# lachinov/brats2019

Measured on AMD Instinct MI355X. Metric: volumes_per_sec_fwd_bwd_128cubed_x4ch, higher is better.
Workload: dtype bf16

## Files before the change

### brats2019_amd/_lib.py

```python
from __future__ import annotations

import ctypes as C
import os

import torch

_PKG = os.path.dirname(os.path.abspath(__file__))
LIB_PATH = os.environ.get("RU_LIB_PATH") or os.path.join(_PKG, "lib", "libresunet_hip.so")

_lib = None
PRECISIONS = {"f32": 0, "bf16x3": 1}
GRAD_PRECISIONS = {"bf16x3": 1, "bf16": 2}
FUSE_GN_BWD_STATS, FUSE_GN_BWD_APPLY, FUSE_SIDE_STREAM, FUSE_BATCH_WREDUCE, FUSE_TAIL_FINALIZE, FUSE_PW_DGRAD = 1, 2, 4, 8, 16, 32

_vp, _f, _d, _i, _sz = C.c_void_p, C.c_float, C.c_double, C.c_int, C.c_size_t

SIGNATURES = {
    "ru_last_error": (C.c_char_p, []),
    "ru_version": (_i, []),
    "ru_device_ok": (_i, []),
    "ru_conv3d_workspace_bytes": (_sz, [_i] * 7),
    "ru_conv3d_fwd": (_i, [_vp, _vp, _vp, _vp] + [_i] * 7 + [_vp, _sz, _vp]),
    "ru_conv3d_bwd_data": (_i, [_vp, _vp, _vp] + [_i] * 7 + [_vp, _sz, _vp]),
    "ru_conv3d_fwd_p": (_i, [_vp, _vp, _vp, _vp] + [_i] * 8 + [_vp, _sz, _vp]),
# ... 48 lines not shown
    "ru_comm_destroy": (_i, [_vp]),
    "ru_comm_rank": (_i, [_vp]),
    "ru_comm_world": (_i, [_vp]),
    "ru_allreduce": (_i, [_vp, _vp, _sz, _i, _vp]),
    "ru_comm_group_begin": (_i, []),
    "ru_comm_group_end": (_i, []),
    "ru_tta_merge": (_i, [_vp, _i, C.c_uint, _vp, _vp, _vp, _i, _i, _i, _i, _vp]),
    "ru_compose_labels": (_i, [_vp, _vp, C.c_ulonglong, _vp, _sz, _vp]),
    "ru_dice_counts": (_i, [_vp, _vp, _vp, _i, _i, _sz, _vp]),
    "ru_dice_accumulate": (_i, [_vp, _vp, _i, _i, _i, _vp]),
    "ru_hausdorff_workspace_bytes": (_sz, [_i] * 6),
    "ru_hausdorff_sq": (_i, [_vp, _vp] + [_i] * 6 + [_vp, _vp, _sz, _vp]),
    "ru_hausdorff_accumulate": (_i, [_vp, _vp] + [_i] * 4 + [_vp]),
    "ru_label_confusion": (_i, [_vp, _vp, _i, _i, _i, _sz, _vp, _vp, _vp]),
    "ru_overlap_accumulate": (_i, [_vp, _i, _i, _i, _i, _vp, _vp, _vp]),
    "ru_dice1d_accumulate": (_i, [_vp, _vp, _i, _i, _i, _vp]),
    "ru_rmse_accumulate": (_i, [_vp, _vp, _vp]),
    "ru_tile_gather": (_i, [_vp, _vp] + [_i] * 6 + [C.POINTER(_i), _i, _i, _i, _vp]),
    "ru_tile_scatter": (_i, [_vp, _vp] + [_i] * 6 + [C.POINTER(_i), _i, _i, _i, C.POINTER(_i), C.POINTER(_i), _vp]),
    "ru_case_bbox": (_i, [_vp, _vp, _i, _i, _i, _i, _vp]),
    "ru_case_workspace_bytes": (_sz, [_i, _i, _i, _i]),
    "ru_case_stats": (_i, [_vp, _vp, _i, _i, _i, _i, C.POINTER(_i), C.POINTER(_i), _vp, _sz, _vp]),
    "ru_case_prepare": (_i, [_vp, _vp, _vp, _i, _i, _i, _i, C.POINTER(_i), C.POINTER(_i), C.POINTER(_i), C.POINTER(_i), _i, C.c_uint, _vp]),
    "ru_tta_merge_box": (_i, [_vp, _i, C.c_uint, _vp, _vp, _vp, _i, _i, _i, _i, C.POINTER(_i), C.POINTER(_i), _vp]),
    "ru_cc_workspace_bytes": (_sz, [_i, _i, _i]),
    "ru_cc_reject": (_i, [_vp, _i, _i, _i, _d, _vp, _sz, _vp]),
    "ru_paste_labels": (_i, [_vp, _vp, _i, _i, _i, C.POINTER(_i), C.POINTER(_i), _vp]),
    "ru_zscore_workspace_bytes": (_sz, [_i, _sz]),
    "ru_zscore_stats": (_i, [_vp, _vp, _i, _sz, _vp, _sz, _vp]),
    "ru_augment_patch": (_i, [_vp, _vp, _vp, _vp, _i, _i, _i, _i, _vp, _vp, _vp, _i, _vp, _vp, _vp, _vp, _vp]),
    "ru_layout_convert": (_i, [_vp, _vp, _i, _i, _sz, _i, _vp]),
    "ru_upsample2x_trilinear_fwd_l": (_i, [_vp, _vp] + [_i] * 5 + [_f, _vp]),
    "ru_upsample2x_trilinear_bwd_l": (_i, [_vp, _vp] + [_i] * 5 + [_vp]),
    "ru_conv3d_fwd_l": (_i, [_vp, _vp, _vp, _vp] + [_i] * 7 + [_vp, _sz, _vp]),
    "ru_conv3d_bwd_weight_l": (_i, [_vp, _vp, _vp] + [_i] * 7 + [_vp, _sz, _vp]),
}


CRIT_KINDS = {"Dice_loss_joint": 0, "BCE_Loss": 1, "MSE_Loss": 2, "CE_Loss": 3, "Dice1D": 4, "GDL_joint": 5, "sens_loss_joint": 6,
              "Dice_loss_separate": 7}
CRIT_MOMENTS, CRIT_MAX_TERMS = 7, 8
CRIT_MASK_LOGS, CRIT_MASK_ALL = (1 << 4) | (1 << 5), 0x7F
CRIT_M_D2 = 6

CONF_PROB, CONF_LABEL, OVERLAP_MAX_LABELS = 0, 1, 8
OVERLAP_MODES = {"itk": 0, "wt": 1, "validate": 2}


class CritTerm(C.Structure):
    _fields_ = [("kind", _i), ("weight", _d), ("priority", _d), ("bg_weight", _d)]


def load():
    global _lib
    if _lib is not None:
        return _lib
    if not os.path.exists(LIB_PATH):
        raise RuntimeError(
            "libresunet_hip.so not found at %s -- build it with `python -m brats2019_amd.build` "
            "(hipcc, gfx950).  There is no CPU fallback for this path." % LIB_PATH)
    lib = C.CDLL(LIB_PATH)
    for name, (res, args) in SIGNATURES.items():
        if os.environ.get("RU_LIB_PATH") and not hasattr(lib, name):
            continue
        fn = getattr(lib, name)
        fn.restype = res
# ... 45 lines not shown
```

### brats2019_amd/csrc/engine.hip

```cpp
#include "ru_common.h"

#include <vector>
#include <math.h>
#include <stdlib.h>
#include <string.h>

#include <string>
#include <vector>

namespace ru {

static thread_local char g_err[512] = "";
void set_error(const char* fmt, ...) {
    va_list ap;
    va_start(ap, fmt);
    vsnprintf(g_err, sizeof(g_err), fmt, ap);
    va_end(ap);
}
int hip_fail(hipError_t e, const char* what) {
    set_error("%s: %s", what, hipGetErrorString(e));
    return RU_EHIP;
}

constexpr float kSlope = 1e-2f;
// ... 614 lines not shown
    }
    const float* cur = stem_fused ? h->y0 : h->t0;
    h->first_s.assign(h->first_blocks.size(), BlockSave());
    for (size_t j = 0; j < h->first_blocks.size(); ++j) {
        rc = block_fwd(h, params, A, s, h->first_blocks[j], cur, N, Dl[0], Hl[0], Wl[0], h->first_s[j], &cur, (stem_fused && j == 0) ? &h->g0 : nullptr);
        if (rc) return rc;
    }
    h->skips.assign(depth - 1, nullptr);
    h->enc_s.assign(depth - 1, {});
    for (int i = 0; i < depth - 1; ++i) {
        h->skips[i] = cur;
        h->enc_s[i].assign(h->enc_blocks[i].size(), BlockSave());
        for (size_t j = 0; j < h->enc_blocks[i].size(); ++j) {
            const int lv = j == 0 ? i : i + 1;
            rc = block_fwd(h, params, A, s, h->enc_blocks[i][j], cur, N, Dl[lv], Hl[lv], Wl[lv], h->enc_s[i][j], &cur);
            if (rc) return rc;
        }
    }
    h->dstage.assign(depth - 1, DecSave());
    h->dec_s.assign(depth - 1, {});
    for (int i = depth - 2; i >= 0; --i) {
        DecSave& ds = h->dstage[i];
        ds.level = i;
        ds.z = cur;
        ds.skip = h->skips[i];
        const int Ci = h->ch[i], Cc = h->ch[i + 1];
        const bool recycle = !h->training;
        float* c_early = recycle ? A.alloc((size_t)N * Ci * Vl(i)) : nullptr;
        const size_t dmark = A.off;
        if (!h->c16) {
            ds.u = A.alloc((size_t)N * Cc * Vl(i));
            RU_RUN(up2_fwd_launch(cur, ds.u, N, Cc, Dl[i + 1], Hl[i + 1], Wl[i + 1], s));
        }
        ds.v = A.alloc((size_t)N * Ci * Vl(i));
        Conv1Args c1{};
        c1.x0 = ds.u; c1.C0 = Cc; c1.y = ds.v; c1.out_slope = kSlope;
        c1.N = N; c1.Cout = Ci; c1.V = Vl(i);
        ds.c = recycle ? c_early : A.alloc((size_t)N * Ci * Vl(i));
        Conv1Args c2{};
        c2.x0 = ds.skip; c2.C0 = Ci; c2.x1 = ds.v; c2.C1 = Ci;
        c2.y = ds.c; c2.out_slope = 1.f; c2.N = N; c2.Cout = Ci; c2.V = Vl(i);
        if (h->c16) {
            float* zc = A.alloc((size_t)N * Ci * Vl(i + 1));
            c1.x0 = cur; c1.y = zc; c1.out_slope = 1.f; c1.V = Vl(i + 1);
            c1.wT = P(h, params, h->up_w[i]); c1.ldw = Cc;
            RU_RUN(conv1_16_launch(c1, s));
            RU_RUN(up2_fwd16_launch(zc, ds.v, N, Ci, Dl[i + 1], Hl[i + 1], Wl[i + 1], kSlope, s));
            c2.wT = P(h, params, h->dec1_w[i]); c2.ldw = 2 * Ci;
            RU_RUN(conv1_16_launch(c2, s));
        } else {
            c1.wT = h->pack + h->pk_upT[i]; c1.ldw = Ci;
            RU_RUN(conv1_launch(c1, s));
            c2.wT = h->pack + h->pk_decT[i]; c2.ldw = Ci;
            RU_RUN(conv1_launch(c2, s));
        }
        if (recycle) A.rewind(dmark);
        cur = ds.c;
        h->dec_s[i].assign(h->dec_blocks[i].size(), BlockSave());
        for (size_t j = 0; j < h->dec_blocks[i].size(); ++j) {
            const bool defer = i == 0 && j + 1 == h->dec_blocks[i].size() && h->c16 &&
                               (h->precision == RU_PREC_BF16X3 ? conv3_sb_head_takes_residual(N, C0, h->nout, Dl[0], Hl[0], Wl[0])
                                                               : (!h->training && conv3_f32c_head_takes_residual(C0, h->nout, Wl[0])));
            rc = block_fwd(h, params, A, s, h->dec_blocks[i][j], cur, N, Dl[i], Hl[i], Wl[i], h->dec_s[i][j], &cur, nullptr, defer);
            if (rc) return rc;
            if (defer) head_block = &h->dec_s[i][j];
        }
    }
    h->head_in = cur;
    t_hint_c = C0;
    float* pdst = probs_out;
    h->probs = probs_out;
    Conv3Args a{};
    a.x = cur; a.wp = h->pack + h->pk_out; a.bias = P(h, params, h->conv_out_b); a.y = pdst; a.sigmoid = 1;
    a.mode = h->precision; a.wfrag = h->fpack + h->fk_out; a.in_c16 = h->c16;
    a.N = N; a.Cin = C0; a.Cout = h->nout; a.D = Dl[0]; a.H = Hl[0]; a.W = Wl[0];
    if (head_block) {
        a.x = head_block->y2; a.in_scale = head_block->g2.scale; a.in_shift = head_block->g2.shift; a.in_slope = kSlope; a.in_res = head_block->x;
        a.in_sum_out = head_block->out;
    }
    RU_RUN(conv3_launch(a, s));
    if (!A.dry) { h->packed_params = h->training ? nullptr : params; h->packed_base = h->pack; h->packed_prec = h->precision; h->packed_c16 = h->c16; h->pack_sig = conv3_sb_switch_signature(); }
    return RU_OK;
// ... 828 lines not shown

extern "C" int ru_tta_merge(const float* probs, int K, unsigned flips, float* mean_out, unsigned char* mask, unsigned long long* counts,
                            int C, int D, int H, int W, ru_stream_t stream) {
    RU_REQUIRE(probs && mask && counts, "ru_tta_merge: null argument");
    return tta_merge_launch(probs, K, flips, mean_out, mask, counts, C, D, H, W, (hipStream_t)stream);
}
extern "C" int ru_compose_labels(const unsigned char* mask, const unsigned long long* counts, unsigned long long et_min, unsigned char* labels,
                                 size_t V, ru_stream_t stream) {
    RU_REQUIRE(mask && counts && labels, "ru_compose_labels: null argument");
    return compose_labels_launch(mask, counts, et_min, labels, V, (hipStream_t)stream);
}

extern "C" int ru_dice_accumulate(const unsigned long long* counts, double* acc, int N, int C, int nacc, ru_stream_t stream) {
    return dice_accumulate_launch(counts, acc, N, C, nacc, (hipStream_t)stream);
}
extern "C" int ru_dice_counts(const float* p, const float* g, unsigned long long* counts, int N, int C, size_t V, ru_stream_t stream) {
    RU_REQUIRE(p && g && counts && N > 0 && C > 0, "ru_dice_counts: bad argument");
    return dice_counts_launch(p, g, counts, N * C, V, (hipStream_t)stream);
}

extern "C" int ru_layout_convert(const float* src, float* dst, int N, int C, size_t V, int to_c16, ru_stream_t stream) {
    RU_REQUIRE(src && dst && N > 0, "ru_layout_convert: bad argument");
    return layout_convert_launch(src, dst, N, C, V, to_c16, (hipStream_t)stream);
}

extern "C" int ru_upsample2x_trilinear_fwd_l(const float* x, float* y, int N, int C, int D, int H, int W, float out_slope, ru_stream_t stream) {
    RU_REQUIRE(x && y && N > 0 && C > 0 && D > 0 && H > 0 && W > 0, "ru_upsample2x_trilinear_fwd_l: bad argument");
    return up2_fwd16_launch(x, y, N, C, D, H, W, out_slope, (hipStream_t)stream);
}
extern "C" int ru_upsample2x_trilinear_bwd_l(const float* dy, float* dx, int N, int C, int D, int H, int W, ru_stream_t stream) {
    RU_REQUIRE(dy && dx && N > 0 && C > 0 && D > 0 && H > 0 && W > 0, "ru_upsample2x_trilinear_bwd_l: bad argument");
    return up2_bwd16_launch(dy, dx, N, C, D, H, W, (hipStream_t)stream);
}
extern "C" int ru_conv3d_fwd_l(const float* x, const float* w, const float* bias, float* y, int N, int Cin, int Cout, int D, int H, int W,
                               int flags, void* ws, size_t ws_bytes, ru_stream_t stream) {
    RU_REQUIRE(x && w && y, "ru_conv3d_fwd_l: null argument");
    hipStream_t s = (hipStream_t)stream;
    WsCarver C(ws, ws_bytes);
    Conv3Args a{};
    void* wf = C.take(conv3_sb_frag_bytes(Cin, Cout) / 4 + 64);
    RU_WS_OK(C);
    const bool f32 = (flags & 16) != 0;
    a.products = (flags & 32) ? 2 : 0;
    RU_REQUIRE(!f32 || ((flags & 3) != 0 && !(flags & (4 | 8))), "ru_conv3d_fwd_l: the exact-f32 form needs a voxel-major side and takes neither the 4-channel copy nor a split-form input");
    const bool gop = (flags & 64) && !f32 && (flags & 3) == 3 && !(flags & (4 | 8)) && !bias && conv3_mxg_usable(N, Cin, Cout, D, H, W);
    int rc = f32 ? conv3_f32c_pack_weights(w, wf, Cin, Cout, 0, s) : conv3_sb_pack_weights(w, wf, Cin, Cout, 0, s, gop);
    if (rc) return rc;
    a.mode = f32 ? RU_PREC_F32 : RU_PREC_BF16X3; a.wfrag = wf;
    a.in_c16 = flags & 1; a.out_c16 = (flags >> 1) & 1;
    a.in_s16 = (flags >> 3) & 1;
    RU_REQUIRE(!a.in_s16 || a.in_c16, "ru_conv3d_fwd_l: the split form is a voxel-major layout");
    a.x = x; a.bias = bias; a.y = y; a.N = N; a.Cin = Cin; a.Cout = Cout; a.D = D; a.H = H; a.W = W;
    if (gop) {
        const size_t nvox = (size_t)N * D * H * W;
        float* g16 = C.take(nvox * 16);
        RU_WS_OK(C);
        rc = conv3_mxg_split_launch(x, g16, nvox, s);
        if (rc) return rc;
        a.x = g16; a.in_s16 = 1; a.in_g16 = 1; a.products = 0;
    }
    if (flags & 4) {
        RU_REQUIRE(!(flags & 1) && conv3_sb4_usable(N, Cin, Cout, D, H, W), "ru_conv3d_fwd_l: shape does not fit the 4-channel kernel");
        const size_t V = (size_t)D * H * W;
        float* x4 = C.take((size_t)N * 4 * V);
        void* wf4 = C.take(conv3_sb4_frag_bytes(Cout) / 4 + 64);
        RU_WS_OK(C);
// ... 44 lines not shown
```

### brats2019_amd/csrc/pointwise_c16.hip

```cpp
#include "pw_helpers.hpp"
#include "fin_tail.hpp"
#include <type_traits>
#include <stdlib.h>

namespace ru {

typedef float f32x4_c16 __attribute__((ext_vector_type(4)));
template <int I, int N, class F> __device__ __forceinline__ void static_for_c1_impl(F&& f) {
    if constexpr (I < N) { f(std::integral_constant<int, I>{}); static_for_c1_impl<I + 1, N>(f); }
}
template <int N, class F> __device__ __forceinline__ void static_for_c1(F&& f) { static_for_c1_impl<0, N>(f); }

static inline dim3 c16_grid(size_t V, int blocks_nc, unsigned cap = 2048) {
    size_t bx = (V * 4 + 255) / 256;
    if (bx > cap) bx = cap;
    if (bx < 1) bx = 1;
    return dim3((unsigned)bx, (unsigned)blocks_nc);
}

template <int RES, bool NT = false>
__global__ __launch_bounds__(256) void gn_apply16_kernel(const float* __restrict__ x, const float* __restrict__ scale, const float* __restrict__ shift,
                                                         const float* __restrict__ res, float* __restrict__ y, int C, size_t V, float slope,
                                                         const float* __restrict__ rscale, const float* __restrict__ rshift, float rslope) {
    const int nb = blockIdx.y, CB = C >> 4;
// ... 164 lines not shown
        pw_split8(o, hi, lo);
        op[v * 4 + hf] = hi;
        op[v * 4 + 2 + hf] = lo;
    }
}
int gn_bwd_apply16_launch(const float* x, const float* dy, const float* scale, const float* shift, const float* coef, float slope, float* dx,
                          int N, int C, size_t V, int split, hipStream_t s) {
    RU_REQUIRE(C % 16 == 0, "gn_bwd_apply16: C must be a multiple of 16");
    if (split) {
        size_t bx = (V * 2 + 255) / 256;
        if (bx > 2048) bx = 2048;
        hipLaunchKernelGGL(gn_bwd_apply16_split_kernel, dim3((unsigned)bx, (unsigned)(N * (C / 16))), dim3(256), 0, s, x, dy, scale, shift, coef, slope, dx, C, V);
    } else {
        hipLaunchKernelGGL(gn_bwd_apply16_kernel, c16_grid(V, N * (C / 16)), dim3(256), 0, s, x, dy, scale, shift, coef, slope, dx, C, V);
    }
    RU_CHECK_LAUNCH("gn_bwd_apply16_kernel");
    return RU_OK;
}

__global__ __launch_bounds__(256) void up2_fwd16_kernel(const float* __restrict__ x, float* __restrict__ y, int D, int H, int W, float slope) {
    const int Do = 2 * D, Ho = 2 * H, Wo = 2 * W;
    const size_t nb = blockIdx.y;
    const size_t Vi = (size_t)D * H * W, Vo = Vi * 8;
    const float4* xp = reinterpret_cast<const float4*>(x) + nb * Vi * 4;
    float4* yp = reinterpret_cast<float4*>(y) + nb * Vo * 4;
    const bool nt_out = (size_t)gridDim.y * Vo * 16 * sizeof(float) >= ((size_t)128 << 20);
    const size_t total = (size_t)(D + 1) * (H + 1) * Wo * 4;
    for (size_t f = (size_t)blockIdx.x * 256 + threadIdx.x; f < total; f += (size_t)gridDim.x * 256) {
        const int q = (int)(f & 3);
        size_t r = f >> 2;
        const int xo = (int)(r % Wo); r /= Wo;
        const int ky = (int)(r % (H + 1)) - 1;
        const int kz = (int)(r / (H + 1)) - 1;
        int x0, x1; float lx0, lx1;
        up2_src(xo, W, x0, x1, lx0, lx1);
        const int zA = kz < 0 ? 0 : kz, zB = kz + 1 > D - 1 ? D - 1 : kz + 1;
        const int yA = ky < 0 ? 0 : ky, yB = ky + 1 > H - 1 ? H - 1 : ky + 1;
        const size_t rAA = ((size_t)zA * H + yA) * W, rAB = ((size_t)zA * H + yB) * W, rBA = ((size_t)zB * H + yA) * W, rBB = ((size_t)zB * H + yB) * W;
        const float4 a00 = xp[(rAA + x0) * 4 + q], b00 = xp[(rAA + x1) * 4 + q];
        const float4 a01 = xp[(rAB + x0) * 4 + q], b01 = xp[(rAB + x1) * 4 + q];
        const float4 a10 = xp[(rBA + x0) * 4 + q], b10 = xp[(rBA + x1) * 4 + q];
        const float4 a11 = xp[(rBB + x0) * 4 + q], b11 = xp[(rBB + x1) * 4 + q];
        float4 e00, e01, e10, e11;
#define RU_UPX(c) e00.c = lx0 * a00.c + lx1 * b00.c; e01.c = lx0 * a01.c + lx1 * b01.c; e10.c = lx0 * a10.c + lx1 * b10.c; e11.c = lx0 * a11.c + lx1 * b11.c
        RU_UPX(x); RU_UPX(y); RU_UPX(z); RU_UPX(w);
#undef RU_UPX
#pragma unroll
        for (int dz = 0; dz < 2; ++dz) {
            const int zo = 2 * kz + 1 + dz;
            if (zo < 0 || zo >= Do) continue;
            int z0, z1; float lz0, lz1;
            up2_src(zo, D, z0, z1, lz0, lz1);
#pragma unroll
            for (int dy = 0; dy < 2; ++dy) {
                const int yo = 2 * ky + 1 + dy;
                if (yo < 0 || yo >= Ho) continue;
                int y0, y1; float ly0, ly1;
                up2_src(yo, H, y0, y1, ly0, ly1);
                float4 o;
#define RU_UP2(c) o.c = lrelu(lz0 * (ly0 * e00.c + ly1 * e01.c) + lz1 * (ly0 * e10.c + ly1 * e11.c), slope)
                RU_UP2(x); RU_UP2(y); RU_UP2(z); RU_UP2(w);
#undef RU_UP2
                if (nt_out) __builtin_nontemporal_store(f32x4_c16{o.x, o.y, o.z, o.w}, reinterpret_cast<f32x4_c16*>(yp + (((size_t)zo * Ho + yo) * Wo + xo) * 4 + q));
                else yp[(((size_t)zo * Ho + yo) * Wo + xo) * 4 + q] = o;
            }
        }
    }
}
int up2_fwd16_launch(const float* x, float* y, int N, int C, int D, int H, int W, float slope, hipStream_t s) {
    RU_REQUIRE(C % 16 == 0, "up2_fwd16: C must be a multiple of 16");
    const size_t total = (size_t)(D + 1) * (H + 1) * (2 * W) * 4;
    size_t bx = (total + 255) / 256;
    if (bx > 16384) bx = 16384;
    hipLaunchKernelGGL(up2_fwd16_kernel, dim3((unsigned)bx, (unsigned)(N * (C / 16))), dim3(256), 0, s, x, y, D, H, W, slope);
    RU_CHECK_LAUNCH("up2_fwd16_kernel");
    return RU_OK;
}

#ifndef RU_UP2B_ZC
#define RU_UP2B_ZC 8
#endif
constexpr int UP2B_ZC = RU_UP2B_ZC;
__global__ __launch_bounds__(256) void up2_bwd16_kernel(const float* __restrict__ dy, float* __restrict__ dx, int D, int H, int W) {
    const int Do = 2 * D, Ho = 2 * H, Wo = 2 * W;
    const size_t nb = blockIdx.y;
    const size_t Vi = (size_t)D * H * W, Vo = Vi * 8;
    const float4* dp = reinterpret_cast<const float4*>(dy) + nb * Vo * 4;
    float4* op = reinterpret_cast<float4*>(dx) + nb * Vi * 4;
    const int nch = (D + UP2B_ZC - 1) / UP2B_ZC;
    const size_t total = (size_t)nch * H * W * 4;
    for (size_t f = (size_t)blockIdx.x * 256 + threadIdx.x; f < total; f += (size_t)gridDim.x * 256) {
        const int q = (int)(f & 3);
        size_t r = f >> 2;
        const int kx = (int)(r % W); r /= W;
        const int ky = (int)(r % H);
        const int k0 = (int)(r / H) * UP2B_ZC;
        const int k1 = k0 + UP2B_ZC < D ? k0 + UP2B_ZC : D;
        float wy[4], wx[4];
        size_t oy[4], ox[4];
#pragma unroll
        for (int t = 0; t < 4; ++t) {
            const int y = 2 * ky - 1 + t, xx = 2 * kx - 1 + t;
            wy[t] = (y >= 0 && y < Ho) ? up2_coef(y, H, ky) : 0.f;
            wx[t] = (xx >= 0 && xx < Wo) ? up2_coef(xx, W, kx) : 0.f;
            oy[t] = (size_t)(y < 0 ? 0 : (y >= Ho ? Ho - 1 : y)) * Wo;
            ox[t] = (size_t)(xx < 0 ? 0 : (xx >= Wo ? Wo - 1 : xx)) * 4 + q;
        }
        float4 accP = make_float4(0.f, 0.f, 0.f, 0.f), accC = accP;
// ... 426 lines not shown
```

### brats2019_amd/csrc/pw_helpers.hpp

```cpp
#pragma once
#include "ru_common.h"

namespace ru {

__device__ __forceinline__ float wave_sum(float v) {
#pragma unroll
    for (int o = 32; o > 0; o >>= 1) v += __shfl_xor(v, o);
    return v;
}
__device__ __forceinline__ double wave_sum_d(double v) {
#pragma unroll
    for (int o = 32; o > 0; o >>= 1) v += __shfl_xor(v, o);
    return v;
}
__device__ __forceinline__ float block_sum(float v, float* buf) {
    v = wave_sum(v);
    __syncthreads();
    if ((threadIdx.x & 63) == 0) buf[threadIdx.x >> 6] = v;
    __syncthreads();
    return buf[0] + buf[1] + buf[2] + buf[3];
}
__device__ __forceinline__ double block_sum_d(double v, double* buf) {
    v = wave_sum_d(v);
    __syncthreads();
    if ((threadIdx.x & 63) == 0) buf[threadIdx.x >> 6] = v;
    __syncthreads();
    return buf[0] + buf[1] + buf[2] + buf[3];
}
__device__ __forceinline__ float lrelu(float v, float slope) { return v > 0.f ? v : v * slope; }

static inline unsigned grid1d(size_t n, int per_block, unsigned cap = 1u << 20) {
    size_t b = (n + per_block - 1) / per_block;
    if (b < 1) b = 1;
    return (unsigned)(b > cap ? cap : b);
}

typedef __bf16 pw_bf16x2 __attribute__((ext_vector_type(2)));
typedef unsigned int pw_u32x4 __attribute__((ext_vector_type(4)));
__device__ __forceinline__ void pw_split8(const float (&t)[8], pw_u32x4& hi, pw_u32x4& lo) {
    split_n<4>(t, hi, lo);
}

__device__ __forceinline__ void up2_src(int o, int n, int& i0, int& i1, float& l0, float& l1) {
    float src = 0.5f * (float)o - 0.25f;
    if (src < 0.f) src = 0.f;
    i0 = (int)src;
    l1 = src - (float)i0;
    l0 = 1.f - l1;
    i1 = i0 + (i0 < n - 1 ? 1 : 0);
}

__device__ __forceinline__ float up2_coef(int o, int n, int k) {
    int i0, i1; float l0, l1;
    up2_src(o, n, i0, i1, l0, l1);
    return (i0 == k ? l0 : 0.f) + (i1 == k ? l1 : 0.f);
}

}
```

### brats2019_amd/csrc/ru_common.h

```cpp
#pragma once
#include <hip/hip_runtime.h>
#include <stddef.h>
#include <stdint.h>
#include <stdio.h>
#include <stdarg.h>

#include <vector>

#include "../../include/resunet_hip.h"

namespace ru {

typedef __bf16 ru_bf16x2 __attribute__((ext_vector_type(2)));
__device__ __forceinline__ void split_pair(float a, float b, unsigned& hb, unsigned& lb) {
    ru_bf16x2 h;
    h[0] = (__bf16)a;
    h[1] = (__bf16)b;
    hb = __builtin_bit_cast(unsigned, h);
    const float h0 = __builtin_bit_cast(float, __builtin_amdgcn_perm(hb, hb, 0x01000c0cu));
    const float h1 = __builtin_bit_cast(float, hb & 0xffff0000u);
    ru_bf16x2 l;
    l[0] = (__bf16)(a - h0);
    l[1] = (__bf16)(b - h1);
    lb = __builtin_bit_cast(unsigned, l);
// ... 258 lines not shown
                    int N, int C, size_t V, float slope, hipStream_t s);
int gn_bwd_tiles(size_t V);
int gn_bwd_reduce_launch(const float* x, const float* dy, const float* scale, const float* shift, const float* mean,
                         const float* rstd, float slope, float* partials, int N, int C, size_t V, int G, hipStream_t s);
int gn_bwd_finalize_launch(const float* partials, int nblk, const float* gamma, const float* mean, const float* rstd,
                           float* coef, float* dgamma, float* dbeta, int N, int C, size_t V, int G, hipStream_t s, int s2_sign = 0);
bool conv3_sb_bst_usable(int N, int Cout, int D, int H, int W);
int gn_bwd_apply_launch(const float* x, const float* dy, const float* scale, const float* shift, const float* coef,
                        float slope, float* dx, int N, int C, size_t V, hipStream_t s);

int lrelu_fwd_launch(const float* x, float* y, size_t n, float slope, hipStream_t s);
int lrelu_bwd_launch(const float* y, const float* dy, float* dx, size_t n, float slope, hipStream_t s);
int sigmoid_launch(const float* x, float* y, size_t n, hipStream_t s);
int sigmoid_bwd_launch(const float* p, const float* dp, float* dz, size_t n, hipStream_t s);
int add_launch(const float* a, const float* b, float* y, size_t n, hipStream_t s);
int fill_launch(float* p, float v, size_t n, hipStream_t s);
int up2_fwd_launch(const float* x, float* y, int N, int C, int D, int H, int W, hipStream_t s);
int up2_bwd_launch(const float* dy, float* dx, int N, int C, int D, int H, int W, hipStream_t s);
int bias_grad_launch(const float* dy, float* db, int N, int C, size_t V, void* ws, size_t ws_bytes, hipStream_t s);
size_t bias_grad_workspace_bytes(int N, int C, size_t V);
int head_grad_c4_launch(const float* p, const float* dp, float* d4, float* db, int N, int C, size_t V, void* ws, size_t ws_bytes, hipStream_t s);
struct CritGradArgs { const float* target; const double* sums; double count; float w_dice, w_bce, bgw, priority; };
int head_grad_c4_crit_launch(const float* p, const CritGradArgs& cg, float* d4, float* db, int N, int C, size_t V, void* ws, size_t ws_bytes, hipStream_t s);

int gn_apply16_launch(const float* x, const float* scale, const float* shift, const float* res, float* y, int N, int C, size_t V, float slope, hipStream_t s,
                      const float* rscale = nullptr, const float* rshift = nullptr, float rslope = 1.f);
int gn_bwd_tiles16(size_t V);
int gn_bwd_reduce16_launch(const float* x, const float* dy, const float* scale, const float* shift, const float* mean, const float* rstd,
                           float slope, float* partials, int N, int C, size_t V, int G, hipStream_t s, const FinTail* fin = nullptr);
int gn_bwd_apply16_launch(const float* x, const float* dy, const float* scale, const float* shift, const float* coef, float slope, float* dx,
                          int N, int C, size_t V, int split, hipStream_t s);
int up2_fwd16_launch(const float* x, float* y, int N, int C, int D, int H, int W, float slope, hipStream_t s);
int up2_bwd16_launch(const float* dy, float* dx, int N, int C, int D, int H, int W, hipStream_t s);
int pack_down16_launch(const float* w, float* wd, float* wdT, int Cout, int Cin, hipStream_t s);
int conv1_16_launch(const Conv1Args& a, hipStream_t s);

int crit_tiles(size_t total);
int crit_sums_launch(const float* p, const float* g, double* sums, int N, int C, size_t V, float bgw, void* ws, size_t ws_bytes, hipStream_t s);
int crit_grad_launch(const float* p, const float* g, const double* sums, double count, float w_dice, float w_bce,
                     float bgw, float priority, float* dp, int N, int C, size_t V, hipStream_t s);
int crit_value_launch(const double* sums, int C, double count, double priority, double w_dice, double w_bce, double* out3, hipStream_t s);
int tta_merge_launch(const float* p, int K, unsigned flips, float* mean_out, unsigned char* mask, unsigned long long* counts, int C, int D, int H, int W, hipStream_t s);
int compose_labels_launch(const unsigned char* mask, const unsigned long long* counts, unsigned long long et_min, unsigned char* labels, size_t V, hipStream_t s);
int dice_counts_launch(const float* p, const float* g, unsigned long long* counts, int rows, size_t V, hipStream_t s);
int dice_accumulate_launch(const unsigned long long* counts, double* acc, int N, int C, int nacc, hipStream_t s);
constexpr int RU_AUG_MAXC = 8;
struct AugmentArgs {
    const float* image;
    const unsigned char* label;
    float* data;
    float* target;
    int C, D, H, W;
    int lo[3], P[3];
    double scale[3];
    int flags;
    float mean[RU_AUG_MAXC], istd[RU_AUG_MAXC], gain[RU_AUG_MAXC], bias[RU_AUG_MAXC];
};
size_t zscore_workspace_bytes(int C, size_t V);
int zscore_stats_launch(const float* x, double* stats, int C, size_t V, void* ws, size_t ws_bytes, hipStream_t s);
int augment_patch_launch(const AugmentArgs& a, hipStream_t s);
int adam_launch(float* w, const float* g, float* m, float* v, float* vmax, size_t n, float lr, float b1, float b2,
                float eps, float wd, int step, hipStream_t s);

}
```

### brats2019_amd/ops.py

```python
from __future__ import annotations

import ctypes as C

import torch

from . import _lib as L

LEAKY_SLOPE = 1e-2


def _dims5(x):
    if x.dim() != 5:
        raise ValueError("expected an NCDHW tensor, got shape %s" % (tuple(x.shape),))
    return [int(v) for v in x.shape]


def _prep(t):
    L.require_gpu()
    if t is None:
        return None
    return t.contiguous().float() if (not t.is_contiguous() or t.dtype != torch.float32) else t


def conv3d(x, w, bias=None, precision="f32"):
# ... 424 lines not shown
    x = _prep(x)
    n, c, d, h, w = _dims5(x)
    y = torch.empty((n, c // 16, d, h, w, 16), dtype=torch.float32, device=x.device)
    L.check(L.load().ru_layout_convert(L.f32(x), L.f32(y), n, c, d * h * w, 1, L.stream()), "ru_layout_convert")
    return y


def from_c16(x):
    x = _prep(x)
    n, cb, d, h, w, _ = (int(v) for v in x.shape)
    y = torch.empty((n, cb * 16, d, h, w), dtype=torch.float32, device=x.device)
    L.check(L.load().ru_layout_convert(L.f32(x), L.f32(y), n, cb * 16, d * h * w, 0, L.stream()), "ru_layout_convert")
    return y


def upsample2x_c16(x, out_slope=1.0):
    x = _prep(x)
    n, cb, d, h, w, _ = (int(v) for v in x.shape)
    y = torch.empty((n, cb, 2 * d, 2 * h, 2 * w, 16), dtype=torch.float32, device=x.device)
    L.check(L.load().ru_upsample2x_trilinear_fwd_l(L.f32(x), L.f32(y), n, cb * 16, d, h, w, float(out_slope), L.stream()),
            "ru_upsample2x_trilinear_fwd_l")
    return y


def upsample2x_bwd_c16(dy):
    dy = _prep(dy)
    n, cb, d2, h2, w2, _ = (int(v) for v in dy.shape)
    dx = torch.empty((n, cb, d2 // 2, h2 // 2, w2 // 2, 16), dtype=torch.float32, device=dy.device)
    L.check(L.load().ru_upsample2x_trilinear_bwd_l(L.f32(dy), L.f32(dx), n, cb * 16, d2 // 2, h2 // 2, w2 // 2, L.stream()),
            "ru_upsample2x_trilinear_bwd_l")
    return dx


def to_split_c16(x_c16):
    hi = x_c16.to(torch.bfloat16)
    lo = (x_c16 - hi.to(torch.float32)).to(torch.bfloat16)
    return torch.cat([hi, lo], dim=-1).contiguous().view(torch.float32)


def conv3d_layout(x, w, bias=None, in_c16=False, out_c16=False, few_channels=False, in_split=False, exact_f32=False, activations=False, gradient=False):
    x, w, bias = _prep(x), _prep(w), _prep(bias)
    if in_c16:
        n, cb, d, h, wd, _ = (int(v) for v in x.shape)
        cin = cb * 16
    else:
        n, cin, d, h, wd = _dims5(x)
    cout = int(w.shape[0])
    y = torch.empty((n, cout // 16, d, h, wd, 16) if out_c16 else (n, cout, d, h, wd), dtype=torch.float32, device=x.device)
    lib = L.load()
    ws = L.workspace(lib.ru_conv3d_workspace_bytes(n, cin, cout, d, h, wd, 3) + (n * d * h * wd * 16 + 65536 if few_channels else 0)
                     + (n * d * h * wd * 64 + 65536 if gradient else 0), x.device)
    L.check(lib.ru_conv3d_fwd_l(L.f32(x), L.f32(w), L.ptr(bias, True), L.f32(y), n, cin, cout, d, h, wd,
                                int(in_c16) | (int(out_c16) << 1) | (int(few_channels) << 2) | (int(in_split) << 3) | (int(exact_f32) << 4) | (int(activations) << 5) | (int(gradient) << 6),
                                L.ptr(ws), ws.numel(), L.stream()), "ru_conv3d_fwd_l")
    return y


def conv3d_bwd_weight_layout(x, dy, x_c16=False, dy_c16=False):
    x, dy = _prep(x), _prep(dy)
    if x_c16:
        n, cb, d, h, wd, _ = (int(v) for v in x.shape)
        cin = cb * 16
    else:
        n, cin, d, h, wd = _dims5(x)
    cout = int(dy.shape[1]) * 16 if dy_c16 else int(dy.shape[1])
    dw = torch.empty((cout, cin, 3, 3, 3), dtype=torch.float32, device=x.device)
# ... 6 lines not shown
```

### include/resunet_hip.h

```cpp
#ifndef RESUNET_HIP_H_
#define RESUNET_HIP_H_

#include <stddef.h>
#include <stdint.h>

#ifdef __cplusplus
extern "C" {
#endif

#define RU_OK 0
#define RU_EINVAL (-1)
#define RU_ENOMEM (-2)
#define RU_EHIP (-3)
#define RU_ESTATE (-4)

#define RU_PREC_F32 0
#define RU_PREC_BF16X3 1
#define RU_PREC_BF16 2

typedef void* ru_stream_t;
typedef struct ru_unet* ru_unet_t;

const char* ru_last_error(void);
int ru_version(void);
// ... 139 lines not shown
int ru_comm_group_end(void);

int ru_tta_merge(const float* probs, int K, unsigned flips, float* mean_out, unsigned char* mask, unsigned long long* counts,
                 int C, int D, int H, int W, ru_stream_t stream);
int ru_compose_labels(const unsigned char* mask, const unsigned long long* counts, unsigned long long et_min, unsigned char* labels,
                      size_t V, ru_stream_t stream);

int ru_tile_gather(const float* data, float* tiles, int N, int C, int D, int H, int W, int T, const int* origins,
                   int td, int th, int tw, ru_stream_t stream);
int ru_tile_scatter(const float* tiles, float* out, int N, int C, int D, int H, int W, int T, const int* origins,
                    int td, int th, int tw, const int* border, const int* center, ru_stream_t stream);
int ru_case_bbox(const float* image, int* box, int C, int D, int H, int W, ru_stream_t stream);
size_t ru_case_workspace_bytes(int C, int D, int H, int W);
int ru_case_stats(const float* image, double* stats, int C, int D, int H, int W, const int* lo, const int* size,
                  void* ws, size_t ws_bytes, ru_stream_t stream);
int ru_case_prepare(const float* image, const double* stats, float* batch, int C, int D, int H, int W, const int* lo, const int* size,
                    const int* pad_left, const int* padded, int K, unsigned flips, ru_stream_t stream);
int ru_tta_merge_box(const float* probs, int K, unsigned flips, float* mean_out, unsigned char* mask, unsigned long long* counts,
                     int C, int D, int H, int W, const int* lo, const int* size, ru_stream_t stream);
size_t ru_cc_workspace_bytes(int D, int H, int W);
int ru_cc_reject(unsigned char* labels, int D, int H, int W, double ratio, void* ws, size_t ws_bytes, ru_stream_t stream);
int ru_paste_labels(const unsigned char* lab, unsigned char* full, int D, int H, int W, const int* lo, const int* size, ru_stream_t stream);

int ru_layout_convert(const float* src, float* dst, int N, int C, size_t V, int to_c16, ru_stream_t stream);
int ru_conv3d_fwd_l(const float* x, const float* w, const float* bias, float* y,
                    int N, int Cin, int Cout, int D, int H, int W, int flags,
                    void* ws, size_t ws_bytes, ru_stream_t stream);
int ru_conv3d_bwd_weight_l(const float* x, const float* dy, float* dw,
                           int N, int Cin, int Cout, int D, int H, int W, int flags,
                           void* ws, size_t ws_bytes, ru_stream_t stream);

int ru_upsample2x_trilinear_fwd_l(const float* x, float* y, int N, int C, int D, int H, int W, float out_slope, ru_stream_t stream);
int ru_upsample2x_trilinear_bwd_l(const float* dy, float* dx, int N, int C, int D, int H, int W, ru_stream_t stream);

int ru_dice_counts(const float* p, const float* g, unsigned long long* counts, int N, int C, size_t V, ru_stream_t stream);
int ru_dice_accumulate(const unsigned long long* counts, double* acc, int N, int C, int nacc, ru_stream_t stream);

size_t ru_hausdorff_workspace_bytes(int N, int C, int D, int H, int W, int mode);
int ru_hausdorff_sq(const float* p, const float* g, int N, int C, int D, int H, int W, int mode, unsigned long long* out,
                    void* ws, size_t ws_bytes, ru_stream_t stream);
int ru_hausdorff_accumulate(const unsigned long long* sq, double* acc, int N, int K, int nacc, int mode, ru_stream_t stream);

#define RU_CONF_PROB 0
#define RU_CONF_LABEL 1
#define RU_OVERLAP_MAX_LABELS 8
#define RU_OVERLAP_ITK 0
#define RU_OVERLAP_WT 1
#define RU_OVERLAP_VALIDATE 2
int ru_label_confusion(const void* pred, const void* target, int kind, int N, int C, size_t V, unsigned long long* conf,
                       unsigned long long* invalid, ru_stream_t stream);
int ru_overlap_accumulate(const unsigned long long* conf, int N, int L, int mode, int nacc, double* acc, double* out, ru_stream_t stream);
int ru_dice1d_accumulate(const unsigned long long* counts, double* acc, int N, int C, int classes, ru_stream_t stream);
int ru_rmse_accumulate(const double* sums, double* acc, ru_stream_t stream);

size_t ru_zscore_workspace_bytes(int C, size_t V);
int ru_zscore_stats(const float* image, double* stats, int C, size_t V, void* ws, size_t ws_bytes, ru_stream_t stream);
int ru_augment_patch(const float* image, const unsigned char* label, const float* mean, const float* inv_std,
                     int C, int D, int H, int W, const int* crop_lo, const int* patch, const double* scale, int flags,
                     const float* gain, const float* bias, float* data_out, float* target_out, ru_stream_t stream);

#ifdef __cplusplus
}
#endif
#endif
```

Measured before the change: 271.1.

## Fuse decoder trilinear upsample with concat 1x1 conv in c16 forward

Result: no change. 272.4, median of 6 (+0.5%).

```diff
diff --git a/brats2019_amd/_lib.py b/brats2019_amd/_lib.py
--- a/brats2019_amd/_lib.py
+++ b/brats2019_amd/_lib.py
@@ -104,6 +104,7 @@
     "ru_layout_convert": (_i, [_vp, _vp, _i, _i, _sz, _i, _vp]),
     "ru_upsample2x_trilinear_fwd_l": (_i, [_vp, _vp] + [_i] * 5 + [_f, _vp]),
     "ru_upsample2x_trilinear_bwd_l": (_i, [_vp, _vp] + [_i] * 5 + [_vp]),
+    "ru_decoder_up_cat_fwd_l": (_i, [_vp] * 5 + [_i] * 5 + [_f, _i, _vp]),
     "ru_conv3d_fwd_l": (_i, [_vp, _vp, _vp, _vp] + [_i] * 7 + [_vp, _sz, _vp]),
     "ru_conv3d_bwd_weight_l": (_i, [_vp, _vp, _vp] + [_i] * 7 + [_vp, _sz, _vp]),
 }
diff --git a/brats2019_amd/csrc/engine.hip b/brats2019_amd/csrc/engine.hip
--- a/brats2019_amd/csrc/engine.hip
+++ b/brats2019_amd/csrc/engine.hip
@@ -670,7 +670,7 @@
             ds.u = A.alloc((size_t)N * Cc * Vl(i));
             RU_RUN(up2_fwd_launch(cur, ds.u, N, Cc, Dl[i + 1], Hl[i + 1], Wl[i + 1], s));
         }
-        ds.v = A.alloc((size_t)N * Ci * Vl(i));
+        ds.v = (!h->c16 || h->training) ? A.alloc((size_t)N * Ci * Vl(i)) : nullptr;
         Conv1Args c1{};
         c1.x0 = ds.u; c1.C0 = Cc; c1.y = ds.v; c1.out_slope = kSlope;
         c1.N = N; c1.Cout = Ci; c1.V = Vl(i);
@@ -683,9 +683,7 @@
             c1.x0 = cur; c1.y = zc; c1.out_slope = 1.f; c1.V = Vl(i + 1);
             c1.wT = P(h, params, h->up_w[i]); c1.ldw = Cc;
             RU_RUN(conv1_16_launch(c1, s));
-            RU_RUN(up2_fwd16_launch(zc, ds.v, N, Ci, Dl[i + 1], Hl[i + 1], Wl[i + 1], kSlope, s));
-            c2.wT = P(h, params, h->dec1_w[i]); c2.ldw = 2 * Ci;
-            RU_RUN(conv1_16_launch(c2, s));
+            RU_RUN(up2_conv1_16_launch(ds.skip, zc, P(h, params, h->dec1_w[i]), 2 * Ci, ds.c, ds.v, kSlope, N, Ci, Dl[i + 1], Hl[i + 1], Wl[i + 1], s));
         } else {
             c1.wT = h->pack + h->pk_upT[i]; c1.ldw = Ci;
             RU_RUN(conv1_launch(c1, s));
@@ -1580,6 +1578,19 @@
     RU_REQUIRE(dy && dx && N > 0 && C > 0 && D > 0 && H > 0 && W > 0, "ru_upsample2x_trilinear_bwd_l: bad argument");
     return up2_bwd16_launch(dy, dx, N, C, D, H, W, (hipStream_t)stream);
 }
+extern "C" int ru_decoder_up_cat_fwd_l(const float* skip, const float* zc, const float* w, float* c, float* v, int N, int C, int D, int H, int W,
+                                       float slope, int fused, ru_stream_t stream) {
+    RU_REQUIRE(skip && zc && w && c && N > 0 && C > 0 && D > 0 && H > 0 && W > 0, "ru_decoder_up_cat_fwd_l: bad argument");
+    RU_REQUIRE(fused || v, "ru_decoder_up_cat_fwd_l: the two-launch sequence needs the up-sampled tensor v");
+    hipStream_t s = (hipStream_t)stream;
+    if (fused) return up2_conv1_16_launch(skip, zc, w, 2 * C, c, v, slope, N, C, D, H, W, s);
+    const int rc = up2_fwd16_launch(zc, v, N, C, D, H, W, slope, s);
+    if (rc) return rc;
+    Conv1Args a{};
+    a.x0 = skip; a.C0 = C; a.x1 = v; a.C1 = C; a.wT = w; a.ldw = 2 * C;
+    a.y = c; a.out_slope = 1.f; a.N = N; a.Cout = C; a.V = (size_t)D * H * W * 8;
+    return conv1_16_launch(a, s);
+}
 extern "C" int ru_conv3d_fwd_l(const float* x, const float* w, const float* bias, float* y, int N, int Cin, int Cout, int D, int H, int W,
                                int flags, void* ws, size_t ws_bytes, ru_stream_t stream) {
     RU_REQUIRE(x && w && y, "ru_conv3d_fwd_l: null argument");
diff --git a/brats2019_amd/csrc/pointwise_c16.hip b/brats2019_amd/csrc/pointwise_c16.hip
--- a/brats2019_amd/csrc/pointwise_c16.hip
+++ b/brats2019_amd/csrc/pointwise_c16.hip
@@ -220,35 +220,16 @@
         const int xo = (int)(r % Wo); r /= Wo;
         const int ky = (int)(r % (H + 1)) - 1;
         const int kz = (int)(r / (H + 1)) - 1;
-        int x0, x1; float lx0, lx1;
-        up2_src(xo, W, x0, x1, lx0, lx1);
-        const int zA = kz < 0 ? 0 : kz, zB = kz + 1 > D - 1 ? D - 1 : kz + 1;
-        const int yA = ky < 0 ? 0 : ky, yB = ky + 1 > H - 1 ? H - 1 : ky + 1;
-        const size_t rAA = ((size_t)zA * H + yA) * W, rAB = ((size_t)zA * H + yB) * W, rBA = ((size_t)zB * H + yA) * W, rBB = ((size_t)zB * H + yB) * W;
-        const float4 a00 = xp[(rAA + x0) * 4 + q], b00 = xp[(rAA + x1) * 4 + q];
-        const float4 a01 = xp[(rAB + x0) * 4 + q], b01 = xp[(rAB + x1) * 4 + q];
-        const float4 a10 = xp[(rBA + x0) * 4 + q], b10 = xp[(rBA + x1) * 4 + q];
-        const float4 a11 = xp[(rBB + x0) * 4 + q], b11 = xp[(rBB + x1) * 4 + q];
-        float4 e00, e01, e10, e11;
-#define RU_UPX(c) e00.c = lx0 * a00.c + lx1 * b00.c; e01.c = lx0 * a01.c + lx1 * b01.c; e10.c = lx0 * a10.c + lx1 * b10.c; e11.c = lx0 * a11.c + lx1 * b11.c
-        RU_UPX(x); RU_UPX(y); RU_UPX(z); RU_UPX(w);
-#undef RU_UPX
+        const Up2Cell e = up2_cell_x(xp, D, H, W, kz, ky, xo, q);
 #pragma unroll
         for (int dz = 0; dz < 2; ++dz) {
             const int zo = 2 * kz + 1 + dz;
             if (zo < 0 || zo >= Do) continue;
-            int z0, z1; float lz0, lz1;
-            up2_src(zo, D, z0, z1, lz0, lz1);
 #pragma unroll
             for (int dy = 0; dy < 2; ++dy) {
                 const int yo = 2 * ky + 1 + dy;
                 if (yo < 0 || yo >= Ho) continue;
-                int y0, y1; float ly0, ly1;
-                up2_src(yo, H, y0, y1, ly0, ly1);
-                float4 o;
-#define RU_UP2(c) o.c = lrelu(lz0 * (ly0 * e00.c + ly1 * e01.c) + lz1 * (ly0 * e10.c + ly1 * e11.c), slope)
-                RU_UP2(x); RU_UP2(y); RU_UP2(z); RU_UP2(w);
-#undef RU_UP2
+                const float4 o = up2_cell_out(e, zo, yo, D, H, slope);
                 if (nt_out) __builtin_nontemporal_store(f32x4_c16{o.x, o.y, o.z, o.w}, reinterpret_cast<f32x4_c16*>(yp + (((size_t)zo * Ho + yo) * Wo + xo) * 4 + q));
                 else yp[(((size_t)zo * Ho + yo) * Wo + xo) * 4 + q] = o;
             }
@@ -262,6 +243,111 @@
     if (bx > 16384) bx = 16384;
     hipLaunchKernelGGL(up2_fwd16_kernel, dim3((unsigned)bx, (unsigned)(N * (C / 16))), dim3(256), 0, s, x, y, D, H, W, slope);
     RU_CHECK_LAUNCH("up2_fwd16_kernel");
+    return RU_OK;
+}
+
+template <int COB>
+__global__ __launch_bounds__(256) void up2_conv1_16_kernel(const float* __restrict__ skip, const float* __restrict__ zc, const float* __restrict__ w, int ldw,
+                                                           float* __restrict__ c, float* __restrict__ v, float slope, int C, int D, int H, int W,
+                                                           int ntile, int nt_out) {
+    const int lane = threadIdx.x & 63, wave = threadIdx.x >> 6;
+    const int n = blockIdx.z, cog = blockIdx.y;
+    const int r = lane & 15, g = lane >> 4;
+    const int CB = C >> 4;
+    const int Do = 2 * D, Ho = 2 * H, Wo = 2 * W;
+    const int nxt = (Wo + 15) >> 4;
+    const int tile = blockIdx.x * 4 + wave;
+    if (tile >= ntile) return;
+    const int xt = tile % nxt, rr = tile / nxt;
+    const int ky = rr % (H + 1) - 1, kz = rr / (H + 1) - 1;
+    const int xo = xt * 16 + r;
+    const bool xok = xo < Wo;
+    const int xc = xok ? xo : Wo - 1;
+    const size_t Vc = (size_t)D * H * W, Vf = Vc * 8;
+    size_t fv[4];
+    bool ok[4];
+#pragma unroll
+    for (int t = 0; t < 4; ++t) {
+        const int zo = 2 * kz + 1 + (t >> 1), yo = 2 * ky + 1 + (t & 1);
+        ok[t] = xok && zo >= 0 && zo < Do && yo >= 0 && yo < Ho;
+        const int zq = zo < 0 ? 0 : (zo >= Do ? Do - 1 : zo), yq = yo < 0 ? 0 : (yo >= Ho ? Ho - 1 : yo);
+        fv[t] = ((size_t)zq * Ho + yq) * Wo + xc;
+    }
+    const float* wrow[COB];
+#pragma unroll
+    for (int cb = 0; cb < COB; ++cb) {
+        const int cob = cog * COB + cb;
+        wrow[cb] = w + (size_t)((cob < CB ? cob : CB - 1) * 16 + r) * ldw + 4 * g;
+    }
+    f32x4_c16 acc[4][COB];
+#pragma unroll
+    for (int t = 0; t < 4; ++t)
+#pragma unroll
+        for (int cb = 0; cb < COB; ++cb) acc[t][cb] = f32x4_c16{0.f, 0.f, 0.f, 0.f};
+    const bool store_v = v != nullptr && cog == 0;
+    auto mma = [&](int kb, const float4 (&xb)[4]) __attribute__((always_inline)) {
+#pragma unroll
+        for (int cb = 0; cb < COB; ++cb) {
+            const float4 wv = *reinterpret_cast<const float4*>(wrow[cb] + kb * 16);
+#pragma unroll
+            for (int t = 0; t < 4; ++t) {
+                acc[t][cb] = __builtin_amdgcn_mfma_f32_16x16x4f32(wv.x, xb[t].x, acc[t][cb], 0, 0, 0);
+                acc[t][cb] = __builtin_amdgcn_mfma_f32_16x16x4f32(wv.y, xb[t].y, acc[t][cb], 0, 0, 0);
+                acc[t][cb] = __builtin_amdgcn_mfma_f32_16x16x4f32(wv.z, xb[t].z, acc[t][cb], 0, 0, 0);
+                acc[t][cb] = __builtin_amdgcn_mfma_f32_16x16x4f32(wv.w, xb[t].w, acc[t][cb], 0, 0, 0);
+            }
+        }
+    };
+    for (int kb = 0; kb < CB; ++kb) {
+        const float* src = skip + ((size_t)(n * CB + kb) * Vf) * 16 + 4 * g;
+        float4 xb[4];
+#pragma unroll
+        for (int t = 0; t < 4; ++t) xb[t] = *reinterpret_cast<const float4*>(src + fv[t] * 16);
+        mma(kb, xb);
+    }
+    for (int kb = 0; kb < CB; ++kb) {
+        const float4* zp = reinterpret_cast<const float4*>(zc) + (size_t)(n * CB + kb) * Vc * 4;
+        const Up2Cell e = up2_cell_x(zp, D, H, W, kz, ky, xc, g);
+        float4 xb[4];
+#pragma unroll
+        for (int t = 0; t < 4; ++t) xb[t] = up2_cell_out(e, 2 * kz + 1 + (t >> 1), 2 * ky + 1 + (t & 1), D, H, slope);
+        if (store_v) {
+            float* dst = v + ((size_t)(n * CB + kb) * Vf) * 16 + 4 * g;
+#pragma unroll
+            for (int t = 0; t < 4; ++t) {
+                if (!ok[t]) continue;
+                if (nt_out) __builtin_nontemporal_store(f32x4_c16{xb[t].x, xb[t].y, xb[t].z, xb[t].w}, reinterpret_cast<f32x4_c16*>(dst + fv[t] * 16));
+                else *reinterpret_cast<float4*>(dst + fv[t] * 16) = xb[t];
+            }
+        }
+        mma(CB + kb, xb);
+    }
+#pragma unroll
+    for (int t = 0; t < 4; ++t) {
+        if (!ok[t]) continue;
+#pragma unroll
+        for (int cb = 0; cb < COB; ++cb) {
+            const int cob = cog * COB + cb;
+            if (cob >= CB) continue;
+            float* dst = c + ((size_t)(n * CB + cob) * Vf + fv[t]) * 16 + 4 * g;
+            if (nt_out) __builtin_nontemporal_store(acc[t][cb], reinterpret_cast<f32x4_c16*>(dst));
+            else *reinterpret_cast<float4*>(dst) = make_float4(acc[t][cb][0], acc[t][cb][1], acc[t][cb][2], acc[t][cb][3]);
+        }
+    }
+}
+int up2_conv1_16_launch(const float* skip, const float* zc, const float* w, int ldw, float* c, float* v, float slope,
+                        int N, int C, int D, int H, int W, hipStream_t s) {
+    RU_REQUIRE(N > 0 && C > 0 && C % 16 == 0 && D > 0 && H > 0 && W > 0, "up2_conv1_16: bad shape (C must be a multiple of 16)");
+    RU_REQUIRE(ldw >= 2 * C && ldw % 4 == 0, "up2_conv1_16: the weight rows must hold 2C floats at a pitch that is a multiple of 4");
+    const int CB = C / 16, cob = CB >= 4 ? 4 : (CB >= 2 ? 2 : 1);
+    const size_t ntile = (size_t)(D + 1) * (H + 1) * ((2 * W + 15) / 16);
+    RU_REQUIRE(ntile < ((size_t)1 << 31), "up2_conv1_16: volume too large");
+    const dim3 grid((unsigned)((ntile + 3) / 4), (unsigned)cdiv(CB, cob), (unsigned)N);
+    const int nt = (size_t)N * C * D * H * W * 8 * sizeof(float) >= ((size_t)128 << 20) ? 1 : 0;
+    if (cob == 4) hipLaunchKernelGGL(up2_conv1_16_kernel<4>, grid, dim3(256), 0, s, skip, zc, w, ldw, c, v, slope, C, D, H, W, (int)ntile, nt);
+    else if (cob == 2) hipLaunchKernelGGL(up2_conv1_16_kernel<2>, grid, dim3(256), 0, s, skip, zc, w, ldw, c, v, slope, C, D, H, W, (int)ntile, nt);
+    else hipLaunchKernelGGL(up2_conv1_16_kernel<1>, grid, dim3(256), 0, s, skip, zc, w, ldw, c, v, slope, C, D, H, W, (int)ntile, nt);
+    RU_CHECK_LAUNCH("up2_conv1_16_kernel");
     return RU_OK;
 }
 
diff --git a/brats2019_amd/csrc/pw_helpers.hpp b/brats2019_amd/csrc/pw_helpers.hpp
--- a/brats2019_amd/csrc/pw_helpers.hpp
+++ b/brats2019_amd/csrc/pw_helpers.hpp
@@ -50,6 +50,34 @@
     i1 = i0 + (i0 < n - 1 ? 1 : 0);
 }
 
+struct Up2Cell { float4 e00, e01, e10, e11; };
+__device__ __forceinline__ Up2Cell up2_cell_x(const float4* __restrict__ xp, int D, int H, int W, int kz, int ky, int xo, int q) {
+    int x0, x1; float lx0, lx1;
+    up2_src(xo, W, x0, x1, lx0, lx1);
+    const int zA = kz < 0 ? 0 : kz, zB = kz + 1 > D - 1 ? D - 1 : kz + 1;
+    const int yA = ky < 0 ? 0 : ky, yB = ky + 1 > H - 1 ? H - 1 : ky + 1;
+    const size_t rAA = ((size_t)zA * H + yA) * W, rAB = ((size_t)zA * H + yB) * W, rBA = ((size_t)zB * H + yA) * W, rBB = ((size_t)zB * H + yB) * W;
+    const float4 a00 = xp[(rAA + x0) * 4 + q], b00 = xp[(rAA + x1) * 4 + q];
+    const float4 a01 = xp[(rAB + x0) * 4 + q], b01 = xp[(rAB + x1) * 4 + q];
+    const float4 a10 = xp[(rBA + x0) * 4 + q], b10 = xp[(rBA + x1) * 4 + q];
+    const float4 a11 = xp[(rBB + x0) * 4 + q], b11 = xp[(rBB + x1) * 4 + q];
+    Up2Cell e;
+#define RU_UPX(c) e.e00.c = lx0 * a00.c + lx1 * b00.c; e.e01.c = lx0 * a01.c + lx1 * b01.c; e.e10.c = lx0 * a10.c + lx1 * b10.c; e.e11.c = lx0 * a11.c + lx1 * b11.c
+    RU_UPX(x); RU_UPX(y); RU_UPX(z); RU_UPX(w);
+#undef RU_UPX
+    return e;
+}
+__device__ __forceinline__ float4 up2_cell_out(const Up2Cell& e, int zo, int yo, int D, int H, float slope) {
+    int z0, z1, y0, y1; float lz0, lz1, ly0, ly1;
+    up2_src(zo, D, z0, z1, lz0, lz1);
+    up2_src(yo, H, y0, y1, ly0, ly1);
+    float4 o;
+#define RU_UP2(c) o.c = lrelu(lz0 * (ly0 * e.e00.c + ly1 * e.e01.c) + lz1 * (ly0 * e.e10.c + ly1 * e.e11.c), slope)
+    RU_UP2(x); RU_UP2(y); RU_UP2(z); RU_UP2(w);
+#undef RU_UP2
+    return o;
+}
+
 __device__ __forceinline__ float up2_coef(int o, int n, int k) {
     int i0, i1; float l0, l1;
     up2_src(o, n, i0, i1, l0, l1);
diff --git a/brats2019_amd/csrc/ru_common.h b/brats2019_amd/csrc/ru_common.h
--- a/brats2019_amd/csrc/ru_common.h
+++ b/brats2019_amd/csrc/ru_common.h
@@ -314,6 +314,8 @@
                           int N, int C, size_t V, int split, hipStream_t s);
 int up2_fwd16_launch(const float* x, float* y, int N, int C, int D, int H, int W, float slope, hipStream_t s);
 int up2_bwd16_launch(const float* dy, float* dx, int N, int C, int D, int H, int W, hipStream_t s);
+int up2_conv1_16_launch(const float* skip, const float* zc, const float* w, int ldw, float* c, float* v, float slope,
+                        int N, int C, int D, int H, int W, hipStream_t s);
 int pack_down16_launch(const float* w, float* wd, float* wdT, int Cout, int Cin, hipStream_t s);
 int conv1_16_launch(const Conv1Args& a, hipStream_t s);
 
diff --git a/brats2019_amd/ops.py b/brats2019_amd/ops.py
--- a/brats2019_amd/ops.py
+++ b/brats2019_amd/ops.py
@@ -480,6 +480,18 @@
     return dx
 
 
+def decoder_up_cat_c16(skip, zc, w, slope=0.01, fused=True, keep_v=False):
+    skip, zc = _prep(skip), _prep(zc)
+    w = _prep(w).reshape(w.shape[0], -1)
+    n, cb, d, h, wd, _ = (int(s) for s in zc.shape)
+    assert tuple(skip.shape) == (n, cb, 2 * d, 2 * h, 2 * wd, 16) and tuple(w.shape) == (cb * 16, cb * 32)
+    c = torch.empty_like(skip)
+    v = torch.empty_like(skip) if (keep_v or not fused) else None
+    L.check(L.load().ru_decoder_up_cat_fwd_l(L.f32(skip), L.f32(zc), L.f32(w), L.f32(c), L.f32(v) if v is not None else None,
+                                             n, cb * 16, d, h, wd, float(slope), 1 if fused else 0, L.stream()), "ru_decoder_up_cat_fwd_l")
+    return (c, v) if keep_v else c
+
+
 def to_split_c16(x_c16):
     hi = x_c16.to(torch.bfloat16)
     lo = (x_c16 - hi.to(torch.float32)).to(torch.bfloat16)
diff --git a/include/resunet_hip.h b/include/resunet_hip.h
--- a/include/resunet_hip.h
+++ b/include/resunet_hip.h
@@ -195,6 +195,8 @@
 
 int ru_upsample2x_trilinear_fwd_l(const float* x, float* y, int N, int C, int D, int H, int W, float out_slope, ru_stream_t stream);
 int ru_upsample2x_trilinear_bwd_l(const float* dy, float* dx, int N, int C, int D, int H, int W, ru_stream_t stream);
+int ru_decoder_up_cat_fwd_l(const float* skip, const float* zc, const float* w, float* c, float* v, int N, int C, int D, int H, int W,
+                            float slope, int fused, ru_stream_t stream);
 
 int ru_dice_counts(const float* p, const float* g, unsigned long long* counts, int N, int C, size_t V, ru_stream_t stream);
 int ru_dice_accumulate(const unsigned long long* counts, double* acc, int N, int C, int nacc, ru_stream_t stream);
```
